# hpy666666/ChineseChessAI

Measured on AMD Instinct MI355X. Metric: self-play games/sec @ 50 MCTS sims, higher is better.
Workload: dtype bf16

## Files before the change

chinesechessai_amd/_lib.py:

```python
import ctypes as C
import os
import subprocess
import sys

_HERE = os.path.dirname(os.path.abspath(__file__))
CSRC = os.path.join(_HERE, "csrc")
LIB_PATH = os.path.join(CSRC, "libxq_hip.so")
SOURCES = [os.path.join(CSRC, "xq_engine.hip"), os.path.join(CSRC, "xq_conv.hip"), os.path.join(CSRC, "xq_replay.hip"),
           os.path.join(CSRC, "xq_tower.hip"), os.path.join(CSRC, "xq_policy.hip"), os.path.join(CSRC, "xq_policy_loss.hip")]
HEADERS = [os.path.join(CSRC, "xq_device.hpp"), os.path.join(CSRC, "xq_attack.hpp"), os.path.join(CSRC, "xq_mfma.hpp"), os.path.join(CSRC, "xq_tower_probes.hpp"),
           os.path.join(CSRC, "xq_tower1wa.hpp"), os.path.join(CSRC, "xq_tower1wa_body.inc"), os.path.join(CSRC, "xq_policy_fc1w_body.inc"),
           os.path.join(_HERE, "..", "include", "xq_selfplay.h"), os.path.join(_HERE, "..", "include", "xq_debug.h")]

MAX_MOVES = 128
MAX_PLIES = 70
WINNER_NONE = 2
NO_KING = -1
POLICY_SIZE = 8100
STATE_WORDS = 10
(S_PLAYER, S_MOVE_COUNT, S_WINNER, S_RED_KING, S_BLACK_KING, S_NO_CAPTURE, S_CONSEC_CHECKS, S_REASON,
 S_REASON_SIDE, S_REASON_COUNT) = range(10)
EVAL_PRIORS, EVAL_LOGITS_F32, EVAL_LOGITS_BF16 = 0, 1, 2
PLANES_NONE, PLANES_NCHW_F32, PLANES_NCHW_BF16, PLANES_NHWC16_BF16 = 0, 1, 2, 3
SAMPLE_RECORD_BYTES = 48 + 8 + 4 + 4 + 256 + 256
# ... 95 lines not shown
    "xq_rules_position_key": (C.c_int, [C.c_int, C.c_void_p, C.c_void_p, C.c_void_p]),
    "xq_rules_make_move": (C.c_int, [C.c_int, C.c_void_p, C.c_void_p, C.c_void_p, C.c_void_p, C.c_void_p,
                                     C.c_void_p, C.c_void_p, C.c_int, C.c_void_p, C.c_void_p, C.c_void_p,
                                     C.c_void_p, C.c_void_p, C.c_void_p]),
    "xq_engine_create": (C.c_int, [C.POINTER(Config), C.POINTER(C.c_void_p)]),
    "xq_engine_destroy": (None, [C.c_void_p]),
    "xq_engine_set_stream": (C.c_int, [C.c_void_p, C.c_void_p]),
    "xq_engine_set_pow_table": (C.c_int, [C.c_void_p, C.c_void_p, C.c_int]),
    "xq_engine_new_games": (C.c_int, [C.c_void_p, C.c_void_p]),
    "xq_engine_set_logit_columns": (C.c_int, [C.c_void_p, C.c_void_p, C.c_int]),
    "xq_engine_set_temperature": (C.c_int, [C.c_void_p, C.c_double, C.c_void_p, C.c_int]),
    "xq_engine_set_root_noise": (C.c_int, [C.c_void_p, C.c_double, C.c_double, C.c_uint64]),
    "xq_engine_set_tree_reuse": (C.c_int, [C.c_void_p, C.c_int]),
    "xq_engine_set_virtual_loss": (C.c_int, [C.c_void_p, C.c_int]),
    "xq_engine_leaf_slots": (C.c_int, [C.c_void_p]),
    "xq_engine_tree_stats": (C.c_int, [C.c_void_p, C.c_void_p, C.c_void_p]),
    "xq_engine_read_root_priors": (C.c_int, [C.c_void_p, C.c_void_p]),
    "xq_engine_set_uniforms": (C.c_int, [C.c_void_p, C.c_void_p]),
    "xq_engine_set_roots": (C.c_int, [C.c_void_p, C.c_void_p, C.c_void_p]),
    "xq_engine_search_round": (C.c_int, [C.c_void_p, C.c_int, C.c_int, C.c_void_p, C.c_void_p, C.c_void_p]),
    "xq_engine_eval_hashnet": (C.c_int, [C.c_void_p, C.c_int]),
    "xq_engine_end_search": (C.c_int, [C.c_void_p, C.c_int, C.c_void_p, C.c_void_p]),
    "xq_engine_play_move": (C.c_int, [C.c_void_p]),
    "xq_engine_finalize": (C.c_int, [C.c_void_p]),
    "xq_engine_active_games": (C.c_int, [C.c_void_p, C.c_void_p]),
    "xq_engine_active_games_post": (C.c_int, [C.c_void_p]),
    "xq_engine_active_games_poll": (C.c_int, [C.c_void_p, C.c_void_p, C.c_void_p]),
    "xq_engine_priors_ptr": (C.c_void_p, [C.c_void_p]),
    "xq_engine_values_ptr": (C.c_void_p, [C.c_void_p]),
    "xq_engine_rounds_per_move": (C.c_int, [C.c_void_p]),
    "xq_engine_read_leaves": (C.c_int, [C.c_void_p] * 6),
    "xq_engine_write_priors": (C.c_int, [C.c_void_p] * 3),
    "xq_engine_read_root_visits": (C.c_int, [C.c_void_p] * 4),
    "xq_engine_read_tree": (C.c_int, [C.c_void_p, C.c_int, C.c_int] + [C.c_void_p] * 8),
    "xq_engine_read_games": (C.c_int, [C.c_void_p] * 8),
    "xq_engine_read_samples": (C.c_int, [C.c_void_p] * 9),
    "xq_engine_pack_samples": (C.c_int, [C.c_void_p, C.c_void_p]),
    "xq_engine_set_root_eval_carry": (C.c_int, [C.c_void_p, C.c_int]),
    "xq_engine_roots_not_ready": (C.c_int, [C.c_void_p, C.c_void_p]),
    "xq_engine_set_row_compaction": (C.c_int, [C.c_void_p, C.c_int]),
    "xq_engine_set_leaf_dedupe": (C.c_int, [C.c_void_p, C.c_int]),
    "xq_engine_set_eval_cache": (C.c_int, [C.c_void_p, C.c_int]),
    "xq_engine_eval_cache_stats": (C.c_int, [C.c_void_p, C.c_void_p, C.c_int]),
    "xq_engine_row_map": (C.c_int, [C.c_void_p, C.POINTER(C.c_void_p), C.POINTER(C.c_void_p)]),
    "xq_engine_read_row_history": (C.c_int, [C.c_void_p, C.c_void_p, C.c_int, C.POINTER(C.c_int64), C.c_int]),
    "xq_engine_read_leaf_rows": (C.c_int, [C.c_void_p, C.c_void_p]),
# ... 24 lines not shown
    "xq_replay_encode_batch": (C.c_int, [C.c_void_p, C.c_void_p, C.c_void_p, C.c_int, C.c_void_p, C.c_void_p]),
    "xq_replay_read_records": (C.c_int, [C.c_void_p, C.c_void_p, C.c_void_p, C.c_int, C.c_void_p]),
    "xq_replay_encode_policy_batch": (C.c_int, [C.c_void_p, C.c_void_p, C.c_void_p, C.c_int, C.c_void_p, C.c_int, C.c_double,
                                                C.c_void_p, C.c_int, C.c_void_p] + [C.c_void_p] * 5),
    "xq_policy_loss_f32": (C.c_int, [C.c_void_p, C.c_void_p, C.c_int64, C.c_int, C.c_void_p, C.c_void_p, C.c_void_p, C.c_int,
                                     C.c_void_p, C.c_void_p]),
    "xq_policy_loss_grad_f32": (C.c_int, [C.c_void_p, C.c_void_p, C.c_void_p, C.c_void_p, C.c_void_p, C.c_float, C.c_int,
                                          C.c_void_p, C.c_int64, C.c_int]),
    "xq_engine_profile": (C.c_int, [C.c_void_p, C.c_int]),
    "xq_engine_profile_read": (C.c_int, [C.c_void_p] * 5),
}

_DEBUG_SIGNATURES = {
    "xq_tower_set_variant": (None, [C.c_int]),
    "xq_tower_set_clock_sample": (None, [C.c_void_p]),
    "xq_tower_debug_stamps": (C.c_int, [C.c_void_p] * 9 + [C.c_int, C.c_int, C.c_void_p]),
    "xq_mfma_probe": (C.c_int, [C.c_void_p] * 4 + [C.c_int, C.c_int, C.c_int]),
    "xq_conv3x3_set_variant": (None, [C.c_int]),
    "xq_conv3x3_debug_stamps": (C.c_int, [C.c_int, C.c_int] + [C.c_void_p] * 6 + [C.c_int, C.c_int, C.c_void_p]),
    "xq_engine_set_search_occupancy": (None, [C.c_int]),
    "xq_engine_set_search_stamps": (C.c_int, [C.c_void_p]),
    "xq_engine_read_row_map": (C.c_int, [C.c_void_p, C.c_int, C.c_void_p, C.c_int, C.c_void_p]),
    "xq_policy_fc_set_variant": (None, [C.c_int]),
    "xq_policy_fc_debug_stamps": (C.c_int, [C.c_int, C.c_void_p, C.c_void_p, C.c_void_p, C.c_void_p, C.c_void_p, C.c_int, C.c_int, C.c_int, C.c_void_p]),
    "xq_policy_fc_debug": (C.c_int, [C.c_int] + [C.c_void_p] * 5 + [C.c_int, C.c_int, C.c_int]),
}

EXPORTS = sorted(_SIGNATURES)
DEBUG_EXPORTS = sorted(_DEBUG_SIGNATURES)
ROW_HISTORY = 65536


def lib():
    global _lib
    if _lib is None:
        if not os.path.exists(LIB_PATH):
            try:
                build()
            except Exception as ex:
                raise XqError("libxq_hip.so is not built (%s) and could not be compiled (%s): run "
                              "`python -c 'import __graft_entry__ as g; g.build()'`; the HIP path has no CPU fallback"
                              % (LIB_PATH, ex))
        _preload_torch_hip_runtime()
        L = C.CDLL(LIB_PATH)
        for table in (_SIGNATURES, _DEBUG_SIGNATURES):
            for name, (res, args) in table.items():
# ... 16 lines not shown
```

chinesechessai_amd/csrc/xq_engine.hip:

```cpp
#include "xq_device.hpp"
#include "../../include/xq_selfplay.h"
#include "../../include/xq_debug.h"
#include <hip/hip_runtime.h>
#include <math.h>
#include <stdio.h>
#include <stdlib.h>
#include <string.h>
#include <string>
#include <thread>
#include <vector>

using namespace xq;

struct __align__(16) GameS {
    int8_t  side;
    uint8_t move_count;
    int8_t  winner;
    uint8_t reason;
    int8_t  reason_side;
    uint8_t reason_count;
    int8_t  rk, bk;
    uint8_t nocap, cchk, n_hist, n_root;
    uint8_t done, n_samples, error, n_plies;
};
// ... 1276 lines not shown
    if (tid == 0) {
        E.row_count[0] = base; E.row_count[1] = base1;
        E.row_hist[seq & (ROW_HIST - 1)] = base + base1;
        E.row_hist_net[seq & (ROW_HIST - 1)] = base; E.row_hist_net[ROW_HIST + (seq & (ROW_HIST - 1))] = base1;
    }
}

__global__ __launch_bounds__(64) void k_end_search(Eng E, EvalPair ev)
{
    __shared__ WaveLds L;
    const int g = blockIdx.x;
    const GameS gs = load_gs(E.gs + g);
    if (gs.done) return;
    const Tree T = tree_of(E, g);
    const int root = E.root_node[g];
    if (E.vloss) {
        for (int k = 0; k < E.leaf_slots; k++)
            consume_eval<true>(E, g, g * E.leaf_slots + k, L, T, root, ev, gs.n_plies);
    } else {
        consume_eval<false>(E, g, g, L, T, root, ev, gs.n_plies);
    }
}

__global__ __launch_bounds__(64) void k_play_move(Eng E)
{
    __shared__ WaveLds L;
    const int g = blockIdx.x, lane = XQ_LANE;
    GameS gs = load_gs(E.gs + g);
    if (gs.done) return;
    const Tree T = tree_of(E, g);
    const int root = E.root_node[g];
    const int nc = T.nc[root], first = T.first[root];
    if (nc == 0) { gs.done = 1; store_gs(E.gs + g, gs); return; }

    for (int j = lane; j < nc; j += 64) L.ibuf[j] = (int)T.N[first + j];
    unpack_to_lds(E.board + (size_t)g * 12, L.bd);
    wave_sync();

    const int pair_v = uni((int)E.pairing[g]);
    const bool store = (gs.side == 1) || pair_v == 0;
    if (store) {
        const size_t si = (size_t)g * XQ_MAX_PLIES + gs.n_samples;
        if (lane < 12) E.s_board[si * 12 + lane] = E.board[(size_t)g * 12 + lane];
        for (int j = lane; j < MAXM; j += 64) {
            E.s_moves[si * MAXM + j] = j < nc ? T.mv[first + j] : 0;
            E.s_counts[si * MAXM + j] = j < nc ? (uint16_t)L.ibuf[j] : 0;
        }
        if (lane == 0) { E.s_player[si] = gs.side; E.s_n[si] = (uint8_t)nc; }
    }

    int pick = -1;
    if (lane == 0) {
        if (E.temperature < 0.01) {
            int am = 0;
// ... 54 lines not shown
    store_gs(E.gs + g, gs);
    if (E.eval_carry && !gs.done) {
        const int c = first + pick, n = T.nc[c], fc = T.first[c];
        const int j0 = lane, j1 = lane + 64;
        const uint16_t m0 = j0 < n ? T.mv[fc + j0] : (uint16_t)0, m1 = j1 < n ? T.mv[fc + j1] : (uint16_t)0;
        const float p0 = j0 < n ? T.P[fc + j0] : 0.f, p1 = j1 < n ? T.P[fc + j1] : 0.f;
        const bool same = (j0 >= n || m0 == L.legal[j0]) && (j1 >= n || m1 == L.legal[j1]);
        const bool ok = n != 0 && n == mr.n_legal && __all(same) && pair_v == 0;
        wave_sync();
        if (ok) {
            if (j0 < n) { const int x = 1 + j0; T.N[x] = 0; T.W[x] = 0.0; T.P[x] = p0; T.mv[x] = m0; T.first[x] = 0; T.nc[x] = 0; T.fl[x] = 0; }
            if (j1 < n) { const int x = 1 + j1; T.N[x] = 0; T.W[x] = 0.0; T.P[x] = p1; T.mv[x] = m1; T.first[x] = 0; T.nc[x] = 0; T.fl[x] = 0; }
            if (lane == 0) {
                const int b0 = E.sims < E.leaf_batch ? E.sims : E.leaf_batch;
                T.N[0] = (uint32_t)b0; T.W[0] = 0.0; T.P[0] = 0.f; T.mv[0] = 0; T.first[0] = 1; T.nc[0] = (uint8_t)n; T.fl[0] = 0;
                E.n_nodes[g] = (uint32_t)(1 + n); E.root_node[g] = 0;
            }
        }
        if (lane == 0) {
            E.root_ready[g] = ok ? 1 : 0;
            if (!ok) atomicAdd(E.roots_not_ready, 1);
        }
    }
}

__device__ void finalize_game(const Eng &E, int g, const GameS &gs)
{
    const int lane = XQ_LANE;
    const int winner = gs.winner == WINNER_NONE ? 0 : gs.winner;
    const int len = gs.n_samples;
    for (int i = lane; i < len; i += 64) {
        const size_t si = (size_t)g * XQ_MAX_PLIES + i;
        const int player = E.s_player[si];
        double fr;
        if (winner == 0) fr = len >= 60 ? (player == 1 ? -0.15 : 0.05) : (player == 1 ? -0.1 : 0.1);
        else if (winner == player) fr = 1.0 + (len <= 30 ? 0.5 : len <= 50 ? 0.3 : len <= 70 ? 0.1 : 0.0);
        else fr = len >= 60 ? -1.2 : -1.0;
        const double imm = i < gs.n_plies ? E.step_reward[si] : 0.0;
        const double scaled = imm * 0.01;
        E.s_z[si] = fr + scaled;
    }
}

__global__ __launch_bounds__(64) void k_finalize(Eng E)
{
    const int g = blockIdx.x;
// ... 393 lines not shown
    unsigned active_posted = 0;
    int8_t *stage_boards = nullptr;
    int32_t *stage_state = nullptr;
    uint16_t *stage_rmoves = nullptr;
    int32_t *stage_rvisits = nullptr;
    float *stage_rpriors = nullptr;
    int32_t *stage_rn = nullptr;
    double *uni_all = nullptr; int32_t *slot_game = nullptr, *next_game = nullptr; GameS *out_gs = nullptr;
    int refill_total = 0, refill_cap = 0;
    uint8_t *pair_all = nullptr;
    bool refill_pairs = false;
    uint8_t *pairing_init = nullptr;
    unsigned row_seq = 0;
    bool row_map_fetched = false;
    unsigned dd_tag = 0;
    unsigned ec_epoch = 16, ec_seq = 0;
    int slot_reuse = 0;
    int ec_want = 0;
    bool ec_roots_ok = true;
    int prof = 0;
    unsigned prof_seen = 0;
    std::vector<std::pair<hipEvent_t, hipEvent_t>> ev_search, ev_play;
    size_t ev_search_used = 0, ev_play_used = 0;
    double search_ms = 0, play_ms = 0;
    int64_t search_n = 0, play_n = 0;
};

static void eval_cache_apply(xq_engine *e) { e->E.ec_on = e->ec_roots_ok ? e->ec_want : 0; }
static void eval_cache_age_out(xq_engine *e) { e->ec_epoch += (unsigned)e->E.ec_keep; }

static bool king_caches_true(const int8_t *board, int rk, int bk)
{
    int r = NO_KING, b = NO_KING, nr = 0, nb = 0;
    for (int s = 0; s < 90; s++) {
        if (board[s] == KING) { r = s; nr++; }
        else if (board[s] == -KING) { b = s; nb++; }
    }
    return nr <= 1 && nb <= 1 && r == rk && b == bk;
}

template <class T> static int dalloc(xq_engine *e, T *&p, size_t count)
{
    void *q = nullptr;
    if (hipMalloc(&q, count * sizeof(T) + 64) != hipSuccess) return -1;
    if (hipMemset(q, 0, count * sizeof(T) + 64) != hipSuccess) return -1;
    e->allocs.push_back(q);
// ... 637 lines not shown
extern "C" int xq_engine_end_search2(xq_engine *e, int eval_kind0, const void *ev_a0, const void *ev_v0, int eval_kind1,
                                     const void *ev_a1, const void *ev_v1)
{
    return end_search_impl(e, eval_kind0, ev_a0, ev_v0, eval_kind1, ev_a1, ev_v1, 1);
}

extern "C" int xq_engine_play_move(xq_engine *e)
{
    if (!e) return fail(XQ_E_INVALID, "null engine");
    HIPCHK(hipSetDevice(e->cfg.device));
    std::pair<hipEvent_t, hipEvent_t> *ev = nullptr;
    if (e->prof) {
        ev = next_events(e->ev_play, e->ev_play_used);
        if (ev) HIPCHK(hipEventRecord(ev->first, e->stream));
    }
    if (e->E.eval_carry) HIPCHK(hipMemsetAsync(e->E.roots_not_ready, 0, 4, e->stream));
    e->ec_epoch += 1;
    hipLaunchKernelGGL(k_play_move, dim3(e->E.G), dim3(64), 0, e->stream, e->E);
    HIPCHK(hipGetLastError());
    if (ev) HIPCHK(hipEventRecord(ev->second, e->stream));
    return 0;
}

extern "C" int xq_engine_set_root_eval_carry(xq_engine *e, int enable)
{
    if (!e) return fail(XQ_E_INVALID, "null engine");
    Eng &E = e->E;
    if (enable && (E.tree_reuse || E.vloss || E.noise_eps > 0.0 || E.opponent_mode))
        return fail(XQ_E_INVALID, "root evaluation carry-over cannot be combined with tree reuse, virtual loss, root noise or "
                                  "opponent mode (the carried priors are the mover's network's)");
    HIPCHK(hipSetDevice(e->cfg.device));
    if (enable && !E.root_ready) {
        if (dalloc(e, E.root_ready, (size_t)E.G) || dalloc(e, E.roots_not_ready, (size_t)1)) return fail(XQ_E_HIP, "hipMalloc failed");
    }
    E.eval_carry = enable ? 1 : 0;
    return 0;
}

extern "C" int xq_engine_set_per_slot_reuse(xq_engine *e, int enable, int keep_plies)
{
    if (!e) return fail(XQ_E_INVALID, "null engine");
    if (keep_plies != 2 && keep_plies != 3) return fail(XQ_E_INVALID, "per-slot reuse: keep_plies must be 2 or 3");
    e->ec_epoch += 3;
    e->slot_reuse = enable ? 1 : 0;
    e->E.ec_keep = enable ? keep_plies : 2;
    return 0;
}

extern "C" int xq_engine_roots_not_ready(xq_engine *e, int32_t *n)
{
    if (!e || !n) return fail(XQ_E_INVALID, "null argument");
    if (!e->E.eval_carry) { *n = e->E.G; return 0; }
    HIPCHK(hipSetDevice(e->cfg.device));
    HIPCHK(hipMemcpyAsync(n, e->E.roots_not_ready, 4, hipMemcpyDeviceToHost, e->stream));
    HIPCHK(hipStreamSynchronize(e->stream));
    return 0;
// ... 349 lines not shown
```

chinesechessai_amd/csrc/xq_policy.hip:

```cpp
#include "../../include/xq_selfplay.h"
#include "../../include/xq_debug.h"
#include "xq_mfma.hpp"
#include <atomic>
#include <type_traits>

#ifndef XQ_TOWER_PROBES
#define XQ_TOWER_PROBES 0
#endif

namespace {
using namespace xqm;

constexpr int BM = 256, BN = 192;
constexpr int A_BYTES = BM * 128, W_BYTES = BN * 128, STAGE_BYTES = A_BYTES + W_BYTES;
constexpr int FC_LDS_BYTES = 2 * STAGE_BYTES;

struct FcArgs {
    const uint16_t *act;
    const uint16_t *w;
    const float *bias;
    uint16_t *out;
    int M, N, K, ncol;
    const int32_t *n_rows;
    unsigned long long *stamps;
// ... 164 lines not shown
    const int act_bytes = rows * K2, w_bytes = BN * K2;
    const int gr = (r16 >> 1) & 7;
    const int vfa = (wn * 96 + 8 * (r16 >> 2) + (r16 & 3)) * 128 + ((q ^ gr) << 4);
    const int vfb = (wm * 128 + r16) * 128 + ((q ^ gr) << 4);
    const int ga = 4 * (wave & 1) + ((lane >> 4) & 3), gw = 2 * wave + ((lane >> 4) & 1);
    const int vdma = (lane >> 3) * K2 + (((lane & 7) ^ ga) << 4);
    const int vdmaw = (lane >> 3) * K2 + (((lane & 7) ^ gw) << 4);
    const int vstore = ((wm * 128 + r16) * P.N + wn * 96 + 8 * q) * 2;
    const int vrow = wm * 128 + r16;
    const int vbias = (wn * 96 + 8 * q) * 4;
    unsigned long long *stamp_p = ABL >= 7 ? P.stamps + (size_t)blockIdx.x * 32 : nullptr;
#if XQ_TOWER_PROBES
    if constexpr (ABL == 7) { XQ_FC1W_ASM(XQ_FC1W_BODY_STAMPED); return; }
    if constexpr (ABL == 8) { XQ_FC1W_ASM(XQ_FC1W_BODY_NODMA_STAMPED); return; }
    if constexpr (ABL == 2) { XQ_FC1W_ASM(XQ_FC1W_BODY_FRONT); return; }
    if constexpr (ABL == 3) { XQ_FC1W_ASM(XQ_FC1W_BODY_NODMA); return; }
    if constexpr (ABL == 4) { XQ_FC1W_ASM(XQ_FC1W_BODY_NOMFMA); return; }
    if constexpr (ABL == 5) { XQ_FC1W_ASM(XQ_FC1W_BODY_EVEN); return; }
    if constexpr (ABL == 6) { XQ_FC1W_ASM(XQ_FC1W_BODY_NOMFMA_NOLDS); return; }
#endif
    XQ_FC1W_ASM(XQ_FC1W_BODY);
}

__global__ __launch_bounds__(256) void k_value_head(const uint16_t *__restrict__ hv, const uint16_t *__restrict__ w1,
                                                    const float *__restrict__ b1, const float *__restrict__ w2,
                                                    const float *__restrict__ b2, uint16_t *__restrict__ out, int M,
                                                    const int32_t *__restrict__ n_rows)
{
    constexpr int K = 720, KP = 736;
    if (n_rows) { const int n = *n_rows; M = n < M ? n : M; }
    const int lane = threadIdx.x & 63, r16 = lane & 15, q = lane >> 4;
    const int row0 = (blockIdx.x * 4 + (threadIdx.x >> 6)) * 16;
    if (row0 >= M) return;
    const int row = row0 + r16 < M ? row0 + r16 : M - 1;
    const uint16_t *xr = hv + (size_t)row * K + q * 8;
    const uint16_t *wr = w1 + (size_t)r16 * KP + q * 8;
    f32x4 acc[8];
#pragma unroll
    for (int nt = 0; nt < 8; nt++) acc[nt] = *reinterpret_cast<const f32x4 *>(b1 + nt * 16 + 4 * q);
#pragma unroll 1
    for (int ks = 0; ks < KP / 32; ks++) {
        const bf16x8 x = *reinterpret_cast<const bf16x8 *>(xr + ks * 32);
#pragma unroll
        for (int nt = 0; nt < 8; nt++) {
            const bf16x8 w = *reinterpret_cast<const bf16x8 *>(wr + (size_t)nt * 16 * KP + ks * 32);
            acc[nt] = __builtin_amdgcn_mfma_f32_16x16x32_bf16(w, x, acc[nt], 0, 0, 0);
        }
    }
    float part = 0.f;
#pragma unroll
    for (int nt = 0; nt < 8; nt++) {
        const f32x4 c = *reinterpret_cast<const f32x4 *>(w2 + nt * 16 + 4 * q);
#pragma unroll
        for (int i = 0; i < 4; i++) part += fmaxf(acc[nt][i], 0.f) * c[i];
    }
    part += __shfl_xor(part, 16, 64);
    part += __shfl_xor(part, 32, 64);
    if (q == 0 && row0 + r16 < M) {
        const float v = tanhf(part + b2[0]);
        out[row0 + r16] = (uint16_t)(pack_bf16x2(v, 0.f) & 0xffffu);
    }
}

}

static int g_fc_variant = -1;
extern "C" void xq_policy_fc_set_variant(int v) { g_fc_variant = v; }

static int fc_lds_opt_in()
{
    static std::atomic<uint64_t> done{ 0 };
    int dev = 0;
    if (hipGetDevice(&dev) != hipSuccess || dev < 0 || dev >= 64) return XQ_E_HIP;
    if (done.load(std::memory_order_acquire) >> dev & 1) return 0;
    if (hipFuncSetAttribute(reinterpret_cast<const void *>(&k_policy_fc<0>), hipFuncAttributeMaxDynamicSharedMemorySize,
                            FC_LDS_BYTES) != hipSuccess)
        return XQ_E_HIP;
    if (hipFuncSetAttribute(reinterpret_cast<const void *>(&k_policy_fc1w<0>), hipFuncAttributeMaxDynamicSharedMemorySize,
                            XQ_FC1W_LDS_BYTES) != hipSuccess)
        return XQ_E_HIP;
#if XQ_TOWER_PROBES
    if (hipFuncSetAttribute(reinterpret_cast<const void *>(&k_policy_fc1w<2>), hipFuncAttributeMaxDynamicSharedMemorySize, XQ_FC1W_LDS_BYTES) != hipSuccess ||
        hipFuncSetAttribute(reinterpret_cast<const void *>(&k_policy_fc1w<3>), hipFuncAttributeMaxDynamicSharedMemorySize, XQ_FC1W_LDS_BYTES) != hipSuccess ||
        hipFuncSetAttribute(reinterpret_cast<const void *>(&k_policy_fc1w<4>), hipFuncAttributeMaxDynamicSharedMemorySize, XQ_FC1W_LDS_BYTES) != hipSuccess ||
        hipFuncSetAttribute(reinterpret_cast<const void *>(&k_policy_fc1w<5>), hipFuncAttributeMaxDynamicSharedMemorySize, XQ_FC1W_LDS_BYTES) != hipSuccess ||
        hipFuncSetAttribute(reinterpret_cast<const void *>(&k_policy_fc1w<6>), hipFuncAttributeMaxDynamicSharedMemorySize, XQ_FC1W_LDS_BYTES) != hipSuccess ||
        hipFuncSetAttribute(reinterpret_cast<const void *>(&k_policy_fc1w<7>), hipFuncAttributeMaxDynamicSharedMemorySize, XQ_FC1W_LDS_BYTES) != hipSuccess ||
        hipFuncSetAttribute(reinterpret_cast<const void *>(&k_policy_fc1w<8>), hipFuncAttributeMaxDynamicSharedMemorySize, XQ_FC1W_LDS_BYTES) != hipSuccess)
        return XQ_E_HIP;
    if (hipFuncSetAttribute(reinterpret_cast<const void *>(&k_policy_fc<1>), hipFuncAttributeMaxDynamicSharedMemorySize, FC_LDS_BYTES) != hipSuccess ||
        hipFuncSetAttribute(reinterpret_cast<const void *>(&k_policy_fc<2>), hipFuncAttributeMaxDynamicSharedMemorySize, FC_LDS_BYTES) != hipSuccess)
        return XQ_E_HIP;
#endif
    done.fetch_or(1ull << dev, std::memory_order_release);
    return 0;
}

extern "C" int xq_policy_fc_bf16(void *stream, const void *act, const void *w, const void *bias, void *out, int M, int N, int K,
                                 const void *n_rows_dev)
{
    if (!act || !w || !bias || !out || M <= 0 || N <= 0 || K < 64 || (K & 63) || N % BN) return XQ_E_INVALID;
    if (int rc = fc_lds_opt_in()) return rc;
// ... 37 lines not shown

extern "C" int xq_policy_fc_debug_stamps(int nodma, void *stream, const void *act, const void *w, const void *bias, void *out, int M, int N,
                                         int K, void *stamps_dev)
{
#if XQ_TOWER_PROBES
    if (!act || !w || !bias || !out || !stamps_dev || M <= 0 || N <= 0 || K < 64 || (K & 63) || N % BN) return XQ_E_INVALID;
    if (int rc = fc_lds_opt_in()) return rc;
    FcArgs a{ (const uint16_t *)act, (const uint16_t *)w, (const float *)bias, (uint16_t *)out, M, N, K, N / BN, nullptr,
              (unsigned long long *)stamps_dev };
    const int ntiles = ((M + BM - 1) / BM) * (N / BN);
    const hipStream_t hs = reinterpret_cast<hipStream_t>(stream);
    if (nodma) hipLaunchKernelGGL(k_policy_fc1w<8>, dim3(ntiles), dim3(256), XQ_FC1W_LDS_BYTES, hs, a);
    else hipLaunchKernelGGL(k_policy_fc1w<7>, dim3(ntiles), dim3(256), XQ_FC1W_LDS_BYTES, hs, a);
    return hipGetLastError() == hipSuccess ? 0 : XQ_E_HIP;
#else
    return XQ_E_INVALID;
#endif
}

extern "C" int xq_value_head_bf16(void *stream, const void *hv, const void *w1, const void *b1, const void *w2, const void *b2,
                                  void *values, int n_rows, const void *n_rows_dev)
{
    if (!hv || !w1 || !b1 || !w2 || !b2 || !values || n_rows <= 0) return XQ_E_INVALID;
    hipLaunchKernelGGL(k_value_head, dim3((n_rows + 63) / 64), dim3(256), 0, reinterpret_cast<hipStream_t>(stream),
                       (const uint16_t *)hv, (const uint16_t *)w1, (const float *)b1, (const float *)w2, (const float *)b2,
                       (uint16_t *)values, n_rows, (const int32_t *)n_rows_dev);
    return hipGetLastError() == hipSuccess ? 0 : XQ_E_HIP;
}
```

chinesechessai_amd/engine.py:

```python
import ctypes as C

import numpy as np

from . import _lib
from .chess_env import decode_move, format_end_reason


def check_per_slot_evaluators(evaluator, opponent_evaluator):
    for ev in (evaluator, opponent_evaluator):
        if isinstance(ev, CallbackEvaluator):
            raise _lib.XqError("a CallbackEvaluator cannot take part in a per-slot two-network session (read_leaves does not "
                               "carry the leaf's network): use HashNetEvaluator / TorchNetEvaluator, or the lock-step play()")


def check_reuse_evaluators(evaluator, opponent_evaluator):
    for ev in (evaluator, opponent_evaluator):
        if isinstance(ev, CallbackEvaluator):
            raise _lib.XqError("reuse=True (evaluation cache and root carry-over in a two-network session) cannot be combined "
                               "with a CallbackEvaluator: its network may answer differently for one position")


def check_keep_plies(keep_plies):
    if isinstance(keep_plies, bool) or keep_plies not in (2, 3):
        raise ValueError("keep_plies must be 2 or 3, got %r" % (keep_plies,))
# ... 345 lines not shown

    def set_pairing(self, pairing=None):
        if pairing is not None:
            pairing = normalise_pairing(pairing, self.n_games, True)
        _lib.check(self.L.xq_engine_set_pairing(self.h, _lib.ptr(pairing)))

    def leaf_rows(self):
        rows = np.zeros(self.n_rows, np.int32)
        _lib.check(self.L.xq_engine_read_leaf_rows(self.h, _lib.ptr(rows)))
        return rows

    def roots_not_ready(self):
        n = np.zeros(1, np.int32)
        _lib.check(self.L.xq_engine_roots_not_ready(self.h, _lib.ptr(n)))
        return int(n[0])

    def _evaluate_pair(self, ev0, ev1):
        if isinstance(ev0, HashNetEvaluator) and isinstance(ev1, HashNetEvaluator):
            _lib.check(self.L.xq_engine_eval_hashnet2(self.h, ev0.salt, ev1.salt))
            t = (_lib.EVAL_PRIORS, self.priors_ptr, self.values_ptr)
            return t, t
        return ev0.evaluate(self), ev1.evaluate(self)

    def search(self, evaluator, opponent_evaluator=None, per_slot=False, skip_round0=False):
        if per_slot:
            if opponent_evaluator is None:
                raise _lib.XqError("search(per_slot=True) needs both evaluators")
            check_per_slot_evaluators(evaluator, opponent_evaluator)
            t0 = t1 = (_lib.EVAL_PRIORS, None, None)
            pp = evaluator.planes_ptr() or opponent_evaluator.planes_ptr()
            for r in range(self.rounds):
                _lib.check(self.L.xq_engine_search_round2(self.h, r, t0[0], t0[1], t0[2], t1[0], t1[1], t1[2], pp))
                t0, t1 = self._evaluate_pair(evaluator, opponent_evaluator)
            _lib.check(self.L.xq_engine_end_search2(self.h, t0[0], t0[1], t0[2], t1[0], t1[1], t1[2]))
            return
        kind, a, v = _lib.EVAL_PRIORS, None, None
        if skip_round0:
            a, v = self.priors_ptr, self.values_ptr
        pp = evaluator.planes_ptr()
        for r in range(1 if skip_round0 else 0, self.rounds):
            _lib.check(self.L.xq_engine_search_round(self.h, r, kind, a, v, pp))
            kind, a, v = evaluator.evaluate(self)
        _lib.check(self.L.xq_engine_end_search(self.h, kind, a, v))

    def root_visits(self):
        G = self.n_games
        moves = np.zeros((G, _lib.MAX_MOVES), np.uint16)
        visits = np.zeros((G, _lib.MAX_MOVES), np.int32)
        n = np.zeros(G, np.int32)
        _lib.check(self.L.xq_engine_read_root_visits(self.h, _lib.ptr(moves), _lib.ptr(visits), _lib.ptr(n)))
        return moves, visits, n

    def read_tree(self, game=0):
        nn, root = np.zeros(1, np.int32), np.zeros(1, np.int32)
        _lib.check(self.L.xq_engine_read_tree(self.h, int(game), 0, _lib.ptr(nn), _lib.ptr(root), *([None] * 6)))
        n = int(nn[0])
        t = {"visit_count": np.zeros(n, np.uint32), "value_sum": np.zeros(n, np.float64), "prior": np.zeros(n, np.float32),
             "move": np.zeros(n, np.uint16), "first_child": np.zeros(n, np.uint16), "n_child": np.zeros(n, np.uint8)}
        _lib.check(self.L.xq_engine_read_tree(self.h, int(game), n, _lib.ptr(nn), _lib.ptr(root),
                                              *[_lib.ptr(t[k]) for k in ("visit_count", "value_sum", "prior", "move", "first_child", "n_child")]))
        t["root"] = int(root[0])
        return t

    def active_games(self):
        n = np.zeros(1, np.int32)
        _lib.check(self.L.xq_engine_active_games(self.h, _lib.ptr(n)))
# ... 75 lines not shown
                    ev.bind(self, net=1, planes_of=evaluator if isinstance(evaluator, TorchNetEvaluator) else None)
                else:
                    ev.bind(self)
        if opponent_evaluator is not None and not (per_slot and self._slot_reuse):
            self.set_eval_cache(False)

    def play(self, evaluator, seeds, opponent_evaluator=None, uniforms=None, check_every=8, read=True,
             temperature_schedule=None):
        carry = self._auto_carry(evaluator, opponent_evaluator)
        self._bind(evaluator, opponent_evaluator)
        self.new_games(seeds)
        if uniforms is not None:
            self.set_uniforms(uniforms)
        self.ply_temperature = []
        cur_t = None
        skip0 = False
        for ply in range(min(self.max_moves, _lib.MAX_PLIES)):
            t = self.temperature if temperature_schedule is None else float(temperature_schedule(ply))
            if temperature_schedule is not None and t != cur_t:
                self.set_temperature(t)
                cur_t = t
            self.ply_temperature.append(t)
            ev = evaluator if (ply % 2 == 0 or opponent_evaluator is None) else opponent_evaluator
            self.search(ev, skip_round0=skip0)
            _lib.check(self.L.xq_engine_play_move(self.h))
            skip0 = carry and not self.row_compaction and self.roots_not_ready() == 0
            if check_every and ply % check_every == check_every - 1:
                if self.active_games_poll() == 0:
                    break
                self.active_games_post()
        _lib.check(self.L.xq_engine_finalize(self.h))
        for ev in (evaluator, opponent_evaluator):
            if ev is not None and hasattr(ev, "after_play"):
                ev.after_play(self)
        return self.read_results() if read else None

    def play_refill(self, evaluator, seeds, records_ptr, check_every=4, max_plies=None, on_ply=None,
                    opponent_evaluator=None, pairing=None, reuse=False):
        seeds = np.ascontiguousarray(seeds, dtype=np.uint32)
        total = len(seeds)
        two = opponent_evaluator is not None
        pairing = normalise_pairing(pairing, total, two)
        if two:
            if reuse:
                check_reuse_evaluators(evaluator, opponent_evaluator)
            check_per_slot_evaluators(evaluator, opponent_evaluator)
        elif self.opponent_mode:
            raise _lib.XqError("play_refill on an opponent-mode engine needs opponent_evaluator")
        reuse = bool(reuse and two)
        if reuse or self._slot_reuse:
            self.set_per_slot_reuse(reuse, keep_plies=(self.reuse_keep_plies or (3 if pairing.any() else 2)) if reuse else 2)
        carry = self._auto_carry(evaluator, opponent_evaluator, reuse=reuse)
        self._bind(evaluator, opponent_evaluator, per_slot=two)
        _lib.check(self.L.xq_engine_refill_begin2(self.h, _lib.ptr(seeds), total, _lib.ptr(pairing)))
        active = np.zeros(1, np.int32)
        plies = 0
        cap = max_plies or (total // self.n_games + 2) * _lib.MAX_PLIES + 8
        skip0 = False
        while plies < cap:
            self.search(evaluator, opponent_evaluator, per_slot=two, skip_round0=skip0)
            _lib.check(self.L.xq_engine_play_move(self.h))
            poll = plies % check_every == check_every - 1
            _lib.check(self.L.xq_engine_refill_step(self.h, C.c_void_p(records_ptr), _lib.ptr(active) if poll else None))
            skip0 = carry and not two and not self.row_compaction and self.roots_not_ready() == 0
            if on_ply is not None:
                on_ply(plies)
            plies += 1
            if poll and int(active[0]) == 0:
                break
        else:
            raise _lib.XqError("play_refill: games still active after %d plies" % cap)
        for ev in (evaluator, opponent_evaluator):
            if ev is not None and hasattr(ev, "after_play"):
                ev.after_play(self)
        out = {k: np.zeros(total, np.int32) for k in ("winner", "reason", "reason_side", "reason_count", "n_plies",
                                                      "n_samples", "error")}
        _lib.check(self.L.xq_engine_refill_read_games(self.h, *[_lib.ptr(out[k]) for k in (
            "winner", "reason", "reason_side", "reason_count", "n_plies", "n_samples", "error")]))
        return out, plies

    def read_results(self):
        G, P, M = self.n_games, _lib.MAX_PLIES, _lib.MAX_MOVES
        b = GameBatch(G, self.temperature)
        b.ply_temperature = list(getattr(self, "ply_temperature", []))
# ... 39 lines not shown
```

include/xq_debug.h:

```cpp
#ifndef XQ_DEBUG_H
#define XQ_DEBUG_H
#include <stdint.h>

#ifdef __cplusplus
extern "C" {
#endif

void xq_tower_set_variant(int variant);

void xq_tower_set_clock_sample(void *dev_u64x3);

int  xq_tower_debug_stamps(void *hip_stream, const void *planes_dev, const void *w1_dev, const void *wt_dev,
                           const void *bias_dev, const void *wh_dev, const void *bh_dev, void *policy_out_dev,
                           void *value_out_dev, int n_boards, int n_blocks, void *stamps_dev);

int  xq_mfma_probe(void *hip_stream, const void *seed64_dev, const void *weights_dev, void *out_dev, int n_workgroups,
                   int iters, int mode);

void xq_conv3x3_set_variant(int variant);

int  xq_conv3x3_debug_stamps(int variant, int ablate, void *hip_stream, const void *x_dev, const void *w_dev,
                             const void *bias_dev, const void *residual_dev, void *y_dev, int n_boards, int relu,
                             void *stamps_dev);

void xq_policy_fc_set_variant(int variant);

int  xq_policy_fc_debug(int ablate, void *hip_stream, const void *act_dev, const void *w_dev, const void *bias_dev, void *out_dev,
                        int n_rows, int n_cols, int k);

int  xq_policy_fc_debug_stamps(int nodma, void *hip_stream, const void *act_dev, const void *w_dev, const void *bias_dev,
                               void *out_dev, int n_rows, int n_cols, int k, void *stamps_dev);

void xq_engine_set_search_occupancy(int waves_per_simd);

int  xq_engine_set_search_stamps(void *dev_u64x16_per_game);

struct xq_engine;
int  xq_engine_read_row_map(struct xq_engine *e, int net, int32_t *row_src_host, int cap, int32_t *count_host);

#ifdef __cplusplus
}
#endif
#endif
```

include/xq_selfplay.h:

```cpp
#ifndef XQ_SELFPLAY_H
#define XQ_SELFPLAY_H
#include <stdint.h>

#ifdef __cplusplus
extern "C" {
#endif

#define XQ_MAX_MOVES    128
#define XQ_MAX_PLIES    70
#define XQ_WINNER_NONE  2
#define XQ_NO_KING      (-1)
#define XQ_POLICY_SIZE  8100

#define XQ_E_INVALID    (-1)
#define XQ_E_HIP        (-2)
#define XQ_E_NOGPU      (-3)
#define XQ_E_STATE      (-4)

enum {
    XQ_R_NONE = 0, XQ_R_KING_CAPTURED = 1, XQ_R_CHECKMATE = 2, XQ_R_REPETITION = 3, XQ_R_FIFTY = 4,
    XQ_R_STALEMATE = 5, XQ_R_PERP_CHECK = 6, XQ_R_PERP_CHASE = 7, XQ_R_MOVE_CAP = 8
};

enum {
// ... 62 lines not shown

int  xq_engine_set_logit_columns(xq_engine *e, const int16_t *map_host, int n_columns);

int  xq_engine_set_temperature(xq_engine *e, double temperature, const double *table_host, int n);
int  xq_engine_set_root_noise(xq_engine *e, double alpha, double epsilon, uint64_t seed);
int  xq_engine_set_tree_reuse(xq_engine *e, int enable);
int  xq_engine_set_virtual_loss(xq_engine *e, int enable);
int  xq_engine_leaf_slots(xq_engine *e);
int  xq_engine_tree_stats(xq_engine *e, int32_t *n_nodes_host , int32_t *pending_visits_host );
int  xq_engine_read_root_priors(xq_engine *e, float *priors_host);

int  xq_engine_set_uniforms(xq_engine *e, const double *uniforms_host );

int  xq_engine_set_roots(xq_engine *e, const int8_t *boards_host, const int32_t *state_host );

int  xq_engine_search_round(xq_engine *e, int round, int eval_kind, const void *eval_a_dev,
                            const void *eval_v_dev, void *planes_dev);

int  xq_engine_eval_hashnet(xq_engine *e, int salt);

int  xq_engine_end_search(xq_engine *e, int eval_kind, const void *eval_a_dev, const void *eval_v_dev);

int  xq_engine_play_move(xq_engine *e);

int  xq_engine_finalize(xq_engine *e);

int  xq_engine_active_games(xq_engine *e, int32_t *n_active_host);
int  xq_engine_active_games_post(xq_engine *e);
int  xq_engine_active_games_poll(xq_engine *e, int32_t *n_active_host, int32_t *ready);

void *xq_engine_priors_ptr(xq_engine *e);
void *xq_engine_values_ptr(xq_engine *e);
int   xq_engine_rounds_per_move(xq_engine *e);

int  xq_engine_read_leaves(xq_engine *e, int8_t *boards_host , int32_t *player_host,
                           uint16_t *moves_host , int32_t *n_moves_host,
                           int32_t *mult_host );
int  xq_engine_write_priors(xq_engine *e, const float *priors_host , const double *values_host);
int  xq_engine_read_root_visits(xq_engine *e, uint16_t *moves_host , int32_t *visits_host,
                                int32_t *n_child_host);
int  xq_engine_read_tree(xq_engine *e, int game, int cap, int32_t *n_nodes_host, int32_t *root_host, uint32_t *visit_count_host,
                         double *value_sum_host, float *prior_host, uint16_t *move_host, uint16_t *first_child_host,
                         uint8_t *n_child_host);
int  xq_engine_read_games(xq_engine *e, int32_t *winner_host, int32_t *reason_host, int32_t *reason_side_host,
                          int32_t *reason_count_host, int32_t *n_plies_host, int32_t *n_samples_host,
                          int32_t *error_host);
// ... 22 lines not shown
int  xq_engine_set_row_compaction(xq_engine *e, int enable);
int  xq_engine_row_map(xq_engine *e, const int32_t **row_src_dev, const int32_t **row_count_dev);
int  xq_engine_read_row_history(xq_engine *e, int32_t *rows_host, int cap, int64_t *n_rounds, int reset);
int  xq_engine_read_leaf_rows(xq_engine *e, int32_t *rows_host );

int  xq_engine_set_leaf_dedupe(xq_engine *e, int enable);

int  xq_engine_set_eval_cache(xq_engine *e, int log2_entries);
int  xq_engine_eval_cache_stats(xq_engine *e, uint64_t *hits_fills_mismatches_host , int reset);

int  xq_engine_refill_begin(xq_engine *e, const uint32_t *seeds_host , int total);
int  xq_engine_refill_step(xq_engine *e, void *records_dev , int32_t *active_host);
int  xq_engine_refill_read_games(xq_engine *e, int32_t *winner, int32_t *reason, int32_t *reason_side,
                                 int32_t *reason_count, int32_t *n_plies, int32_t *n_samples, int32_t *error);
int  xq_engine_refill_read_slots(xq_engine *e, int32_t *slot_game_host );

int  xq_engine_set_pairing(xq_engine *e, const uint8_t *pairing_host );
int  xq_engine_refill_begin2(xq_engine *e, const uint32_t *seeds_host , int total,
                             const uint8_t *pairing_host );
int  xq_engine_search_round2(xq_engine *e, int round, int eval_kind0, const void *eval_a0_dev, const void *eval_v0_dev,
                             int eval_kind1, const void *eval_a1_dev, const void *eval_v1_dev, void *planes_dev);
int  xq_engine_end_search2(xq_engine *e, int eval_kind0, const void *eval_a0_dev, const void *eval_v0_dev,
                           int eval_kind1, const void *eval_a1_dev, const void *eval_v1_dev);
int  xq_engine_row_map_net(xq_engine *e, int net, const int32_t **row_src_dev, const int32_t **row_count_dev);
int  xq_engine_read_row_history_net(xq_engine *e, int net, int32_t *rows_host, int cap, int64_t *n_rounds, int reset);
int  xq_engine_eval_hashnet2(xq_engine *e, int salt0, int salt1);
int  xq_engine_set_per_slot_reuse(xq_engine *e, int enable, int keep_plies);

int  xq_conv3x3_nhwc_bf16(void *hip_stream, const void *x_dev, const void *w_dev, const void *bias_dev,
                          const void *residual_dev, void *y_dev, int n_boards, int c_in, int relu);

int  xq_heads_nhwc_bf16(void *hip_stream, const void *x_dev, const void *w_dev, const void *bias_dev,
                        void *policy_out_dev, void *value_out_dev, int n_boards);

int  xq_tower_nhwc_bf16(void *hip_stream, const void *planes_dev, const void *w1_dev, const void *wt_dev,
                        const void *bias_dev, const void *wh_dev, const void *bh_dev, void *policy_out_dev,
                        void *value_out_dev, int n_boards, int n_blocks, const void *row_src_dev, const void *n_rows_dev);

int  xq_policy_fc_bf16(void *hip_stream, const void *act_dev, const void *w_dev, const void *bias_dev, void *logits_dev,
                       int n_rows, int n_cols, int k, const void *n_rows_dev);

int  xq_value_head_bf16(void *hip_stream, const void *hv_dev, const void *w1_dev, const void *b1_dev, const void *w2_dev,
                        const void *b2_dev, void *values_dev, int n_rows, const void *n_rows_dev);

const char *xq_replay_last_error(void);
int     xq_replay_create(int device, int64_t capacity, void **out);
// ... 26 lines not shown
```

Before: 13440.

## Fuse end-search with play-move and add LDS-staged value head kernel

Merges the final search backup and the move-play step into one kernel launch per ply, removing a launch and a global-memory round trip of game state. The roots_not_ready counter becomes double-buffered so the fused kernel can zero the stale one. Separately, a new value-head kernel stages the first-layer weights through LDS with DMA double-buffering and explicit MFMA/LDS-load interleaving, and it is now the default. Together these add complexity, and the new value head depends on the LDS opt-in call succeeding.

```diff
diff --git a/chinesechessai_amd/_lib.py b/chinesechessai_amd/_lib.py
--- a/chinesechessai_amd/_lib.py
+++ b/chinesechessai_amd/_lib.py
@@ -141,6 +141,8 @@
     "xq_engine_eval_hashnet": (C.c_int, [C.c_void_p, C.c_int]),
     "xq_engine_end_search": (C.c_int, [C.c_void_p, C.c_int, C.c_void_p, C.c_void_p]),
     "xq_engine_play_move": (C.c_int, [C.c_void_p]),
+    "xq_engine_end_search_play": (C.c_int, [C.c_void_p, C.c_int, C.c_void_p, C.c_void_p]),
+    "xq_engine_end_search_play2": (C.c_int, [C.c_void_p, C.c_int, C.c_void_p, C.c_void_p, C.c_int, C.c_void_p, C.c_void_p]),
     "xq_engine_finalize": (C.c_int, [C.c_void_p]),
     "xq_engine_active_games": (C.c_int, [C.c_void_p, C.c_void_p]),
     "xq_engine_active_games_post": (C.c_int, [C.c_void_p]),
@@ -211,6 +213,7 @@
     "xq_engine_set_search_stamps": (C.c_int, [C.c_void_p]),
     "xq_engine_read_row_map": (C.c_int, [C.c_void_p, C.c_int, C.c_void_p, C.c_int, C.c_void_p]),
     "xq_policy_fc_set_variant": (None, [C.c_int]),
+    "xq_value_head_set_variant": (None, [C.c_int]),
     "xq_policy_fc_debug_stamps": (C.c_int, [C.c_int, C.c_void_p, C.c_void_p, C.c_void_p, C.c_void_p, C.c_void_p, C.c_int, C.c_int, C.c_int, C.c_void_p]),
     "xq_policy_fc_debug": (C.c_int, [C.c_int] + [C.c_void_p] * 5 + [C.c_int, C.c_int, C.c_int]),
 }
diff --git a/chinesechessai_amd/csrc/xq_engine.hip b/chinesechessai_amd/csrc/xq_engine.hip
--- a/chinesechessai_amd/csrc/xq_engine.hip
+++ b/chinesechessai_amd/csrc/xq_engine.hip
@@ -1322,14 +1322,9 @@
     }
 }
 
-__global__ __launch_bounds__(64) void k_play_move(Eng E)
-{
-    __shared__ WaveLds L;
-    const int g = blockIdx.x, lane = XQ_LANE;
-    GameS gs = load_gs(E.gs + g);
-    if (gs.done) return;
-    const Tree T = tree_of(E, g);
-    const int root = E.root_node[g];
+__device__ void play_move_game(const Eng &E, int g, GameS gs, const Tree &T, int root, WaveLds &L)
+{
+    const int lane = XQ_LANE;
     const int nc = T.nc[root], first = T.first[root];
     if (nc == 0) { gs.done = 1; store_gs(E.gs + g, gs); return; }
 
@@ -1430,6 +1425,35 @@
             if (!ok) atomicAdd(E.roots_not_ready, 1);
         }
     }
+}
+
+__global__ __launch_bounds__(64) void k_play_move(Eng E)
+{
+    __shared__ WaveLds L;
+    const int g = blockIdx.x;
+    const GameS gs = load_gs(E.gs + g);
+    if (gs.done) return;
+    play_move_game(E, g, gs, tree_of(E, g), E.root_node[g], L);
+}
+
+__global__ __launch_bounds__(64) void k_end_search_play(Eng E, EvalPair ev, int32_t *stale_count)
+{
+    __shared__ WaveLds L;
+    const int g = blockIdx.x;
+    if (g == 0 && XQ_LANE == 0 && stale_count) *stale_count = 0;
+    const GameS gs = load_gs(E.gs + g);
+    if (gs.done) return;
+    const Tree T = tree_of(E, g);
+    const int root = E.root_node[g];
+    if (E.vloss) {
+        for (int k = 0; k < E.leaf_slots; k++)
+            consume_eval<true>(E, g, g * E.leaf_slots + k, L, T, root, ev, gs.n_plies);
+    } else {
+        consume_eval<false>(E, g, g, L, T, root, ev, gs.n_plies);
+    }
+    wave_sync();
+    mem_fence_wave();
+    play_move_game(E, g, gs, T, root, L);
 }
 
 __device__ void finalize_game(const Eng &E, int g, const GameS &gs)
@@ -1869,6 +1893,7 @@
     unsigned prof_seen = 0;
     std::vector<std::pair<hipEvent_t, hipEvent_t>> ev_search, ev_play;
     size_t ev_search_used = 0, ev_play_used = 0;
+    int32_t *roots_not_ready_pair = nullptr;
     double search_ms = 0, play_ms = 0;
     int64_t search_n = 0, play_n = 0;
 };
@@ -2552,6 +2577,47 @@
     return 0;
 }
 
+static int end_search_play_impl(xq_engine *e, int eval_kind, const void *ev_a, const void *ev_v, int eval_kind1, const void *ev_a1,
+                                const void *ev_v1, int two)
+{
+    if (!e || !ev_a || !ev_v || !ev_a1 || !ev_v1) return fail(XQ_E_INVALID, "null argument");
+    if (eval_kind < XQ_EVAL_PRIORS || eval_kind > XQ_EVAL_LOGITS_BF16) return fail(XQ_E_INVALID, "bad eval_kind");
+    if (eval_kind1 < XQ_EVAL_PRIORS || eval_kind1 > XQ_EVAL_LOGITS_BF16) return fail(XQ_E_INVALID, "bad eval_kind");
+    if ((eval_kind != XQ_EVAL_PRIORS || eval_kind1 != XQ_EVAL_PRIORS) && e->E.compact && !e->row_map_fetched)
+        return fail(XQ_E_INVALID, "logits handed in by slot while row compaction is on: fetch xq_engine_row_map or switch it off");
+    if (two) { if (int rc = two_net_ok(e)) return rc; }
+    HIPCHK(hipSetDevice(e->cfg.device));
+    e->E.two_net = two ? 1 : 0;
+    e->E.ec_epoch = e->ec_epoch; e->E.ec_seq = ++e->ec_seq;
+    const EvalPair evp{ { { ev_a, ev_v, eval_kind, 0 }, { ev_a1, ev_v1, eval_kind1, 0 } } };
+    std::pair<hipEvent_t, hipEvent_t> *ev = nullptr;
+    if (e->prof) {
+        ev = next_events(e->ev_play, e->ev_play_used);
+        if (ev) HIPCHK(hipEventRecord(ev->first, e->stream));
+    }
+    int32_t *stale = nullptr;
+    if (e->E.eval_carry) {
+        stale = e->E.roots_not_ready;
+        e->E.roots_not_ready = e->roots_not_ready_pair + (stale == e->roots_not_ready_pair ? 1 : 0);
+    }
+    e->ec_epoch += 1;
+    hipLaunchKernelGGL(k_end_search_play, dim3(e->E.G), dim3(64), 0, e->stream, e->E, evp, stale);
+    HIPCHK(hipGetLastError());
+    if (ev) HIPCHK(hipEventRecord(ev->second, e->stream));
+    return 0;
+}
+
+extern "C" int xq_engine_end_search_play(xq_engine *e, int eval_kind, const void *ev_a, const void *ev_v)
+{
+    return end_search_play_impl(e, eval_kind, ev_a, ev_v, eval_kind, ev_a, ev_v, 0);
+}
+
+extern "C" int xq_engine_end_search_play2(xq_engine *e, int eval_kind0, const void *ev_a0, const void *ev_v0, int eval_kind1,
+                                          const void *ev_a1, const void *ev_v1)
+{
+    return end_search_play_impl(e, eval_kind0, ev_a0, ev_v0, eval_kind1, ev_a1, ev_v1, 1);
+}
+
 extern "C" int xq_engine_set_root_eval_carry(xq_engine *e, int enable)
 {
     if (!e) return fail(XQ_E_INVALID, "null engine");
@@ -2561,7 +2627,8 @@
                                   "opponent mode (the carried priors are the mover's network's)");
     HIPCHK(hipSetDevice(e->cfg.device));
     if (enable && !E.root_ready) {
-        if (dalloc(e, E.root_ready, (size_t)E.G) || dalloc(e, E.roots_not_ready, (size_t)1)) return fail(XQ_E_HIP, "hipMalloc failed");
+        if (dalloc(e, E.root_ready, (size_t)E.G) || dalloc(e, e->roots_not_ready_pair, (size_t)2)) return fail(XQ_E_HIP, "hipMalloc failed");
+        E.roots_not_ready = e->roots_not_ready_pair;
     }
     E.eval_carry = enable ? 1 : 0;
     return 0;
diff --git a/chinesechessai_amd/csrc/xq_policy.hip b/chinesechessai_amd/csrc/xq_policy.hip
--- a/chinesechessai_amd/csrc/xq_policy.hip
+++ b/chinesechessai_amd/csrc/xq_policy.hip
@@ -210,6 +210,24 @@
     XQ_FC1W_ASM(XQ_FC1W_BODY);
 }
 
+__device__ __forceinline__ void value_head_tail(const f32x4 (&acc)[8], const float *__restrict__ w2, const float *__restrict__ b2,
+                                                uint16_t *__restrict__ out, int row0, int r16, int q, int M)
+{
+    float part = 0.f;
+#pragma unroll
+    for (int nt = 0; nt < 8; nt++) {
+        const f32x4 c = *reinterpret_cast<const f32x4 *>(w2 + nt * 16 + 4 * q);
+#pragma unroll
+        for (int i = 0; i < 4; i++) part += fmaxf(acc[nt][i], 0.f) * c[i];
+    }
+    part += __shfl_xor(part, 16, 64);
+    part += __shfl_xor(part, 32, 64);
+    if (q == 0 && row0 + r16 < M) {
+        const float v = tanhf(part + b2[0]);
+        out[row0 + r16] = (uint16_t)(pack_bf16x2(v, 0.f) & 0xffffu);
+    }
+}
+
 __global__ __launch_bounds__(256) void k_value_head(const uint16_t *__restrict__ hv, const uint16_t *__restrict__ w1,
                                                     const float *__restrict__ b1, const float *__restrict__ w2,
                                                     const float *__restrict__ b2, uint16_t *__restrict__ out, int M,
@@ -235,25 +253,83 @@
             acc[nt] = __builtin_amdgcn_mfma_f32_16x16x32_bf16(w, x, acc[nt], 0, 0, 0);
         }
     }
-    float part = 0.f;
-#pragma unroll
-    for (int nt = 0; nt < 8; nt++) {
-        const f32x4 c = *reinterpret_cast<const f32x4 *>(w2 + nt * 16 + 4 * q);
-#pragma unroll
-        for (int i = 0; i < 4; i++) part += fmaxf(acc[nt][i], 0.f) * c[i];
-    }
-    part += __shfl_xor(part, 16, 64);
-    part += __shfl_xor(part, 32, 64);
-    if (q == 0 && row0 + r16 < M) {
-        const float v = tanhf(part + b2[0]);
-        out[row0 + r16] = (uint16_t)(pack_bf16x2(v, 0.f) & 0xffffu);
-    }
+    value_head_tail(acc, w2, b2, out, row0, r16, q, M);
+}
+
+constexpr int VH_CHUNK = 8, VH_NCHUNK = 3, VH_BUF_BYTES = VH_CHUNK * 8 * 1024, VH_LDS_BYTES = 2 * VH_BUF_BYTES;
+
+__global__ __launch_bounds__(256) void k_value_head_wg(const uint16_t *__restrict__ hv, const uint16_t *__restrict__ w1,
+                                                       const float *__restrict__ b1, const float *__restrict__ w2,
+                                                       const float *__restrict__ b2, uint16_t *__restrict__ out, int M,
+                                                       const int32_t *__restrict__ n_rows)
+{
+    constexpr int K = 720, KP = 736, NKS = KP / 32;
+    if (n_rows) { const int n = *n_rows; M = n < M ? n : M; }
+    if ((int)blockIdx.x * 64 >= M) return;
+    const int lane = threadIdx.x & 63, r16 = lane & 15, q = lane >> 4;
+    const int wave = __builtin_amdgcn_readfirstlane(threadIdx.x >> 6);
+    const int row0 = (blockIdx.x * 4 + wave) * 16;
+    const int row = row0 + r16 < M ? row0 + r16 : M - 1;
+    const uint16_t *xr = hv + (size_t)row * K + q * 8;
+    const uint16_t *wr = w1 + (size_t)(wave * 32 + r16) * KP + q * 8;
+
+    auto fetch = [&](int c, int buf) {
+#pragma unroll
+        for (int h = 0; h < 2; h++)
+#pragma unroll
+            for (int k = 0; k < VH_CHUNK; k++)
+                if (c * VH_CHUNK + k < NKS)
+                    dma16_abs(wr + (size_t)h * 16 * KP + (c * VH_CHUNK + k) * 32, buf * VH_BUF_BYTES + (((k * 8 + 2 * wave + h) * 64) << 4));
+    };
+    bf16x8 xs[NKS], wf[2][8];
+#pragma unroll
+    for (int ks = 0; ks < NKS; ks++) xs[ks] = *reinterpret_cast<const bf16x8 *>(xr + ks * 32);
+    fetch(0, 0);
+    fetch(1, 1);
+    f32x4 acc[8];
+#pragma unroll
+    for (int nt = 0; nt < 8; nt++) acc[nt] = *reinterpret_cast<const f32x4 *>(b1 + nt * 16 + 4 * q);
+    const int fbase = lane << 4;
+    auto frags = [&](int slot, int buf, int k) {
+#pragma unroll
+        for (int nt = 0; nt < 8; nt++) wf[slot][nt] = lds_ld128(fbase + buf * VH_BUF_BYTES + (k * 8 + nt) * 1024);
+    };
+    auto compute = [&](int c, int buf) {
+        frags(0, buf, 0);
+        __builtin_amdgcn_sched_barrier(0);
+#pragma unroll
+        for (int k = 0; k < VH_CHUNK; k++)
+            if (c * VH_CHUNK + k < NKS) {
+                const bool more = k + 1 < VH_CHUNK && c * VH_CHUNK + k + 1 < NKS;
+                if (more) frags((k + 1) & 1, buf, k + 1);
+#pragma unroll
+                for (int nt = 0; nt < 8; nt++)
+                    acc[nt] = __builtin_amdgcn_mfma_f32_16x16x32_bf16(wf[k & 1][nt], xs[c * VH_CHUNK + k], acc[nt], 0, 0, 0);
+#pragma unroll
+                for (int nt = 0; nt < 8; nt++) {
+                    if (more) __builtin_amdgcn_sched_group_barrier(0x100, 1, 0);
+                    __builtin_amdgcn_sched_group_barrier(0x008, 1, 0);
+                }
+            }
+    };
+    static_assert(VH_NCHUNK == 3 && VH_NCHUNK * VH_CHUNK >= NKS, "three chunks through two buffers");
+    barrier_dma();
+    compute(0, 0);
+    __syncthreads();
+    fetch(2, 0);
+    compute(1, 1);
+    barrier_dma();
+    compute(2, 0);
+    value_head_tail(acc, w2, b2, out, row0, r16, q, M);
 }
 
 }
 
 static int g_fc_variant = -1;
 extern "C" void xq_policy_fc_set_variant(int v) { g_fc_variant = v; }
+
+static int g_vh_variant = -1;
+extern "C" void xq_value_head_set_variant(int v) { g_vh_variant = (v == 0) ? 0 : -1; }
 
 static int fc_lds_opt_in()
 {
@@ -266,6 +342,9 @@
         return XQ_E_HIP;
     if (hipFuncSetAttribute(reinterpret_cast<const void *>(&k_policy_fc1w<0>), hipFuncAttributeMaxDynamicSharedMemorySize,
                             XQ_FC1W_LDS_BYTES) != hipSuccess)
+        return XQ_E_HIP;
+    if (hipFuncSetAttribute(reinterpret_cast<const void *>(&k_value_head_wg), hipFuncAttributeMaxDynamicSharedMemorySize,
+                            VH_LDS_BYTES) != hipSuccess)
         return XQ_E_HIP;
 #if XQ_TOWER_PROBES
     if (hipFuncSetAttribute(reinterpret_cast<const void *>(&k_policy_fc1w<2>), hipFuncAttributeMaxDynamicSharedMemorySize, XQ_FC1W_LDS_BYTES) != hipSuccess ||
@@ -349,8 +428,14 @@
                                   void *values, int n_rows, const void *n_rows_dev)
 {
     if (!hv || !w1 || !b1 || !w2 || !b2 || !values || n_rows <= 0) return XQ_E_INVALID;
-    hipLaunchKernelGGL(k_value_head, dim3((n_rows + 63) / 64), dim3(256), 0, reinterpret_cast<hipStream_t>(stream),
-                       (const uint16_t *)hv, (const uint16_t *)w1, (const float *)b1, (const float *)w2, (const float *)b2,
-                       (uint16_t *)values, n_rows, (const int32_t *)n_rows_dev);
+    const hipStream_t hs = reinterpret_cast<hipStream_t>(stream);
+    if (g_vh_variant == 0) {
+        hipLaunchKernelGGL(k_value_head, dim3((n_rows + 63) / 64), dim3(256), 0, hs, (const uint16_t *)hv, (const uint16_t *)w1,
+                           (const float *)b1, (const float *)w2, (const float *)b2, (uint16_t *)values, n_rows, (const int32_t *)n_rows_dev);
+    } else {
+        if (int rc = fc_lds_opt_in()) return rc;
+        hipLaunchKernelGGL(k_value_head_wg, dim3((n_rows + 63) / 64), dim3(256), VH_LDS_BYTES, hs, (const uint16_t *)hv, (const uint16_t *)w1,
+                           (const float *)b1, (const float *)w2, (const float *)b2, (uint16_t *)values, n_rows, (const int32_t *)n_rows_dev);
+    }
     return hipGetLastError() == hipSuccess ? 0 : XQ_E_HIP;
 }
diff --git a/chinesechessai_amd/engine.py b/chinesechessai_amd/engine.py
--- a/chinesechessai_amd/engine.py
+++ b/chinesechessai_amd/engine.py
@@ -391,7 +391,7 @@
             return t, t
         return ev0.evaluate(self), ev1.evaluate(self)
 
-    def search(self, evaluator, opponent_evaluator=None, per_slot=False, skip_round0=False):
+    def search(self, evaluator, opponent_evaluator=None, per_slot=False, skip_round0=False, play=False):
         if per_slot:
             if opponent_evaluator is None:
                 raise _lib.XqError("search(per_slot=True) needs both evaluators")
@@ -401,7 +401,8 @@
             for r in range(self.rounds):
                 _lib.check(self.L.xq_engine_search_round2(self.h, r, t0[0], t0[1], t0[2], t1[0], t1[1], t1[2], pp))
                 t0, t1 = self._evaluate_pair(evaluator, opponent_evaluator)
-            _lib.check(self.L.xq_engine_end_search2(self.h, t0[0], t0[1], t0[2], t1[0], t1[1], t1[2]))
+            end2 = self.L.xq_engine_end_search_play2 if play else self.L.xq_engine_end_search2
+            _lib.check(end2(self.h, t0[0], t0[1], t0[2], t1[0], t1[1], t1[2]))
             return
         kind, a, v = _lib.EVAL_PRIORS, None, None
         if skip_round0:
@@ -410,7 +411,7 @@
         for r in range(1 if skip_round0 else 0, self.rounds):
             _lib.check(self.L.xq_engine_search_round(self.h, r, kind, a, v, pp))
             kind, a, v = evaluator.evaluate(self)
-        _lib.check(self.L.xq_engine_end_search(self.h, kind, a, v))
+        _lib.check((self.L.xq_engine_end_search_play if play else self.L.xq_engine_end_search)(self.h, kind, a, v))
 
     def root_visits(self):
         G = self.n_games
@@ -532,8 +533,7 @@
                 cur_t = t
             self.ply_temperature.append(t)
             ev = evaluator if (ply % 2 == 0 or opponent_evaluator is None) else opponent_evaluator
-            self.search(ev, skip_round0=skip0)
-            _lib.check(self.L.xq_engine_play_move(self.h))
+            self.search(ev, skip_round0=skip0, play=True)
             skip0 = carry and not self.row_compaction and self.roots_not_ready() == 0
             if check_every and ply % check_every == check_every - 1:
                 if self.active_games_poll() == 0:
@@ -568,8 +568,7 @@
         cap = max_plies or (total // self.n_games + 2) * _lib.MAX_PLIES + 8
         skip0 = False
         while plies < cap:
-            self.search(evaluator, opponent_evaluator, per_slot=two, skip_round0=skip0)
-            _lib.check(self.L.xq_engine_play_move(self.h))
+            self.search(evaluator, opponent_evaluator, per_slot=two, skip_round0=skip0, play=True)
             poll = plies % check_every == check_every - 1
             _lib.check(self.L.xq_engine_refill_step(self.h, C.c_void_p(records_ptr), _lib.ptr(active) if poll else None))
             skip0 = carry and not two and not self.row_compaction and self.roots_not_ready() == 0
diff --git a/include/xq_debug.h b/include/xq_debug.h
--- a/include/xq_debug.h
+++ b/include/xq_debug.h
@@ -25,6 +25,8 @@
 
 void xq_policy_fc_set_variant(int variant);
 
+void xq_value_head_set_variant(int variant);
+
 int  xq_policy_fc_debug(int ablate, void *hip_stream, const void *act_dev, const void *w_dev, const void *bias_dev, void *out_dev,
                         int n_rows, int n_cols, int k);
 
diff --git a/include/xq_selfplay.h b/include/xq_selfplay.h
--- a/include/xq_selfplay.h
+++ b/include/xq_selfplay.h
@@ -108,6 +108,8 @@
 int  xq_engine_end_search(xq_engine *e, int eval_kind, const void *eval_a_dev, const void *eval_v_dev);
 
 int  xq_engine_play_move(xq_engine *e);
+
+int  xq_engine_end_search_play(xq_engine *e, int eval_kind, const void *eval_a_dev, const void *eval_v_dev);
 
 int  xq_engine_finalize(xq_engine *e);
 
@@ -176,6 +178,8 @@
                              int eval_kind1, const void *eval_a1_dev, const void *eval_v1_dev, void *planes_dev);
 int  xq_engine_end_search2(xq_engine *e, int eval_kind0, const void *eval_a0_dev, const void *eval_v0_dev,
                            int eval_kind1, const void *eval_a1_dev, const void *eval_v1_dev);
+int  xq_engine_end_search_play2(xq_engine *e, int eval_kind0, const void *eval_a0_dev, const void *eval_v0_dev,
+                                int eval_kind1, const void *eval_a1_dev, const void *eval_v1_dev);
 int  xq_engine_row_map_net(xq_engine *e, int net, const int32_t **row_src_dev, const int32_t **row_count_dev);
 int  xq_engine_read_row_history_net(xq_engine *e, int net, int32_t *rows_host, int cap, int64_t *n_rounds, int reset);
 int  xq_engine_eval_hashnet2(xq_engine *e, int salt0, int salt1);
```

Measured after the change: 13490 (median of 6 runs). No clear change (+0.3%).
